# BioinformaticsArchive/POPBAM

Measured on AMD Instinct MI355X. Metric: Msites/sec (nucdiv+sfs+ld, 10kb win, 12 samples) at 1/2/4/8 GPUs, higher is better.
Workload: dtype f64; 1 GPU; configs[2]: synthetic 1 contig x 50 Msites x 12 samples per GPU, consensus call + nucdiv + sfs + ld(ZnS), 10 kb windows; sites_per_gpu=50000000, samples=12, mean_depth=10, window=10000, windows_per_gpu=4999, keys_per_gpu=6000082444, parallelism=dp1 (independent window-range shards, no collective), pieces=1

## Files before the change

popbam_amd/csrc/api.cpp:

```cpp
#include <dlfcn.h>
#include <hip/hip_runtime.h>

#include <algorithm>
#include <cmath>
#include <cstdlib>
#include <cstring>
#include <string>
#include <type_traits>
#include <vector>

#include "pbg_ctx.h"


namespace {

thread_local std::string g_create_error;

int fail(pbg_ctx *c, int code, const std::string &msg) {
    if (c) c->err = msg;
    else g_create_error = msg;
    return code;
}

}

int pbg::ctx_fail(pbg_ctx *c, int code, const std::string &msg) { return fail(c, code, msg); }

namespace {

#define HIPCHK(ctx, expr)                                                                          \
    do {                                                                                           \
        hipError_t _e = (expr);                                                                    \
        if (_e != hipSuccess)                                                                      \
            return fail((ctx), PBG_E_HIP, std::string(#expr) + ": " + hipGetErrorString(_e));      \
    } while (0)

uint32_t rms_of(uint32_t rmsq, int k) {
    const float f = (float)rmsq / (float)k;
    return (uint32_t)((double)std::sqrt(f) + 0.499);
}
uint32_t rms_threshold(int k, int min_rmsQ, int min_depth, int max_depth) {
    if (k < 1 || k < min_depth || k > max_depth) return 0xFFFFFFFFu;
    uint32_t lo = 0, hi = (uint32_t)k * 65025u;
    if ((int)rms_of(hi, k) < min_rmsQ) return 0xFFFFFFFFu;
    while (lo < hi) {
        const uint32_t mid = lo + (hi - lo) / 2;
        if ((int)rms_of(mid, k) >= min_rmsQ) hi = mid;
        else lo = mid + 1;
    }
    return lo;
}

int row_bytes_for(int n) { return n <= 14 ? 2 : n <= 30 ? 4 : n <= 62 ? 8 : 16; }

template <class T>
hipError_t upload(T **dst, const std::vector<T> &v) {
    hipError_t e = hipMalloc((void **)dst, std::max<size_t>(1, v.size()) * sizeof(T));
    if (e != hipSuccess) return e;
    if (v.empty()) return hipSuccess;
    return hipMemcpy(*dst, v.data(), v.size() * sizeof(T), hipMemcpyHostToDevice);
}


}

namespace {
std::vector<int32_t> jsfs_offsets(const pbg::DevParams &dp) {
    std::vector<int32_t> off;
    int32_t at = 0;
    for (int i = 0; i < dp.npops; ++i)
        for (int j = i + 1; j < dp.npops; ++j) {
            off.push_back(at);
            at += (dp.pop_n[i] + 1) * (dp.pop_n[j] + 1);
        }
    off.push_back(at);
    return off;
}

int check_pop_sizes(pbg_ctx *c, const char *what) {
    for (int i = 0; i < c->dp.npops; ++i)
        if (__builtin_popcountll(c->dp.pop_mask[i]) + __builtin_popcountll(c->dp.pop_mask_hi[i]) != c->dp.pop_n[i])
            return fail(c, PBG_E_ARG, std::string(what) + ": pop_n must be the number of samples in pop_mask");
    return PBG_OK;
// ... 187 lines not shown
                    for (uint32_t w = 0; w < 16; ++w)
                        fbeta[pbg::fbeta_index(q, nn, cc, w)] = q ? fk[w] * beta[q << 16 | nn << 8 | cc] : 0.0;
        if ((e = upload(&c->d_fbeta, fbeta)) != hipSuccess) return bad(e, "upload fbeta");
        std::vector<double> lb(pbg::kLbSize, 0.0);
        for (int m = 1; m <= 16; ++m) lb[m] = lb[m - 1] + fk[m - 1];
        for (int d = 3; d <= 16; ++d) {
            double run = 1e300;
            for (int q = 63; q >= 4; --q) {
                for (int cc = 0; cc <= d - 2; ++cc) run = std::min(run, beta[q << 16 | d << 8 | cc]);
                lb[17 + (q - 4) * 17 + d] = run;
            }
        }
        if ((e = upload(&c->d_lb, lb)) != hipSuccess) return bad(e, "upload lb");
        std::vector<double> oe(pbg::kOeSize, 0.0);
        for (int q = 4; q < 64; ++q)
            for (int d = 0; d <= 16; ++d) oe[(q - 4) * 17 + d] = beta[q << 16 | d << 8];
        for (int nn = 0; nn <= 16; ++nn)
            for (int kk = 0; kk <= 16; ++kk) oe[60 * 17 + nn * 17 + kk] = lhet[nn << 8 | kk];
        if ((e = upload(&c->d_oe, oe)) != hipSuccess) return bad(e, "upload one-error tables");
        {
            pbg::ScanTab st{};
            for (int q = 4; q < 64; ++q)
                for (int dd = 3; dd <= 16; ++dd) {
                    const volatile double pe = fk[0] * beta[q << 16 | dd << 8];
                    st.fpe[(q - 4) * 14 + dd - 3] = (float)pe;
                }
            for (int lev = 0; lev < 15; ++lev)
                for (int dd = 3; dd <= 16; ++dd) {
                    const double b = lb[17 + (4 * lev) * 17 + dd];
                    float f = (float)b;
                    if ((double)f > b) f = std::nextafter(f, 0.0f);
                    st.lq[lev * 14 + dd - 3] = f;
                }
            for (int dd = 3; dd <= 16; ++dd) {
                const int idx[4][2] = {{dd, dd - 1}, {dd, 1}, {dd - 1, 0}, {dd - 1, dd - 1}};
                for (int i = 0; i < 4; ++i) {
                    const volatile double h = -4.343 * lhet[idx[i][0] << 8 | idx[i][1]];
                    st.lh[(dd - 3) * 4 + i] = h;
                }
            }
            for (int m = 0; m <= 16; ++m) st.pre[m] = lb[m];
            if ((e = hipMalloc(&c->d_scantab, sizeof(st))) != hipSuccess) return bad(e, "hipMalloc scan tables");
            if ((e = hipMemcpy(c->d_scantab, &st, sizeof(st), hipMemcpyHostToDevice)) != hipSuccess)
                return bad(e, "upload scan tables");
        }
        std::vector<double> bu(60 * 17, 0.0);
        for (int dd = 1; dd <= 16; ++dd) {
            double run = 1e300;
            for (int q = 63; q >= 4; --q) {
                for (int cc = 0; cc <= dd - 1; ++cc) run = std::min(run, beta[q << 16 | dd << 8 | cc]);
                bu[(q - 4) * 17 + dd] = run;
            }
        }
        bool fk_dec = true;
        for (int w = 1; w < 16; ++w) fk_dec = fk_dec && fk[w] <= fk[w - 1];
        for (int i = 0; i < 17 * 3; ++i) d.uni[i] = 255u;
        for (int dd = 1; dd <= 16; ++dd) {
            float h[2];
            for (int t = 0; t < 2; ++t) {
                const float v = (float)(-4.343 * lhet[dd << 8 | (t ? dd : 0)]);
                h[t] = v < 0.0f ? 0.0f : v;
            }
            const float hm[3] = {h[0], h[1], std::min(h[0], h[1])};
            for (int cls = 0; cls < 3; ++cls) {
                uint32_t qthr = 255u;
                for (int q = 63; q >= 4; --q) {
                    const double lbv = lb[dd] * bu[(q - 4) * 17 + dd];
                    if (fk_dec && hm[cls] > 0.0f && lbv * (1.0 - 1e-9) > (double)hm[cls] * (1.0 + 1e-6) + 1e-3) qthr = (uint32_t)q;
                    else break;
                }
                const uint32_t snpq = (uint32_t)(uint64_t)((double)hm[cls] + 0.499) & 0xFFFFu;
                d.uni[dd * 3 + cls] = qthr | snpq << 8;
            }
        }
    }
    std::vector<double> a1, a2, e1, e2;
    pbg::build_sfs_constants(p->n_samples, a1, a2, e1, e2);
    const size_t L = a2.size();
    std::vector<double> sfs(4 * L, 0.0);
    std::copy(a1.begin(), a1.end(), sfs.begin());
    std::copy(a2.begin(), a2.end(), sfs.begin() + L);
    std::copy(e1.begin(), e1.end(), sfs.begin() + 2 * L);
    std::copy(e2.begin(), e2.end(), sfs.begin() + 3 * L);
    if ((e = upload(&c->d_sfs, sfs)) != hipSuccess) return bad(e, "upload sfs constants");
    std::vector<double> r2all;
    for (int i = 0; i < p->n_pops; ++i) {
        std::vector<double> t;
        pbg::build_r2_table(std::max(1, p->pop_n[i]), t);
        c->dt.r2_off[i] = (int32_t)r2all.size();
        r2all.insert(r2all.end(), t.begin(), t.end());
    }
    if ((e = upload(&c->d_r2, r2all)) != hipSuccess) return bad(e, "upload r2 tables");
    if ((e = hipMalloc(&c->d_err, sizeof(int))) != hipSuccess) return bad(e, "hipMalloc err");
    if ((e = hipMemset(c->d_err, 0, sizeof(int))) != hipSuccess) return bad(e, "hipMemset err");
    c->dt.fk = c->d_fk;
    c->dt.beta = c->d_beta;
    c->dt.lhet = c->d_lhet;
    c->dt.fbeta = c->d_fbeta;
    c->dt.lb = c->d_lb;
    c->dt.oe = c->d_oe;
    c->dt.scantab = reinterpret_cast<const uint4 *>(c->d_scantab);
    c->dt.a1 = c->d_sfs;
    c->dt.a2 = c->d_sfs + L;
    c->dt.e1 = c->d_sfs + 2 * L;
    c->dt.e2 = c->d_sfs + 3 * L;
    c->dt.r2 = c->d_r2;
// ... 658 lines not shown
```

popbam_amd/csrc/call_kernel.hip:

```cpp
#include <algorithm>

#include "pbg_common.h"

namespace pbg {
extern const int kBuildKind_call = PBG_BUILD_KIND;
}

namespace pbg {

namespace {

__device__ __forceinline__ unsigned char iupac_rev(unsigned char c) {
    switch (c) {
        case 'A': case 'a': return 0;
        case 'C': case 'c': return 1;
        case 'G': case 'g': return 2;
        case 'T': case 't': return 3;
        default: return 14;
    }
}
__device__ __forceinline__ char iupac_hom(unsigned g) {
    return g == 0 ? 'A' : g == 5 ? 'C' : g == 10 ? 'G' : 'T';
}
__device__ __forceinline__ uint32_t iupac_rev_bf(uint32_t c) {
    const uint32_t i = ((c & 0xDFu) - 'A') & 0xFFu;
    constexpr uint64_t kVal = (1ull << 4) | (2ull << 12) | (3ull << 38);
    constexpr uint32_t kOk = (1u << 0) | (1u << 2) | (1u << 6) | (1u << 19);
    const bool ok = i < 32u && ((kOk >> (i & 31u)) & 1u);
    return ok ? (uint32_t)(kVal >> (2u * (i & 31u))) & 3u : 14u;
}

__device__ __forceinline__ void cswap(uint32_t &a, uint32_t &b) {
    uint32_t hi = a > b ? a : b, lo = a > b ? b : a;
    a = hi;
    b = lo;
}
template <int N>
__device__ __forceinline__ void sortn_desc(uint32_t *k) {
#define CS(i, j) if constexpr ((j) < N) cswap(k[i], k[j])
    CS(0, 1); CS(2, 3); CS(0, 2); CS(1, 3); CS(1, 2); CS(4, 5); CS(6, 7); CS(4, 6);
    CS(5, 7); CS(5, 6); CS(0, 4); CS(2, 6); CS(2, 4); CS(1, 5); CS(3, 7); CS(3, 5);
    CS(1, 2); CS(3, 4); CS(5, 6);
    if constexpr (N <= 8) return;
    CS(8, 9); CS(10, 11); CS(8, 10); CS(9, 11); CS(9, 10);
    CS(12, 13); CS(14, 15); CS(12, 14); CS(13, 15); CS(13, 14); CS(8, 12); CS(10, 14); CS(10, 12);
    CS(9, 13); CS(11, 15); CS(11, 13); CS(9, 10); CS(11, 12); CS(13, 14); CS(0, 8); CS(4, 12);
    CS(4, 8); CS(2, 10); CS(6, 14); CS(6, 10); CS(2, 4); CS(6, 8); CS(10, 12); CS(1, 9);
    CS(5, 13); CS(5, 9); CS(3, 11); CS(7, 15); CS(7, 11); CS(3, 5); CS(7, 9); CS(11, 13);
    CS(1, 2); CS(3, 4); CS(5, 6); CS(7, 8); CS(9, 10); CS(11, 12); CS(13, 14);
#undef CS
}

__device__ __forceinline__ void sort32_desc(uint32_t *k) {
#define CS(i, j) cswap(k[i], k[j])
    CS(0, 1); CS(2, 3); CS(0, 2); CS(1, 3); CS(1, 2); CS(4, 5); CS(6, 7); CS(4, 6);
    CS(5, 7); CS(5, 6); CS(0, 4); CS(2, 6); CS(2, 4); CS(1, 5); CS(3, 7); CS(3, 5);
// ... 291 lines not shown
    a.bsum[0] = slot[0];
    a.bsum[1] = slot[SS];
    a.bsum[2] = slot[2 * SS];
    a.bsum[3] = slot[3 * SS];
    a.cpack = cvalid;
    a.wpack = 0;
    const uint64_t g = likelihood_gl2cns<LHS>(a, k, lhet);
    if constexpr (kRms) return g | rms_word((int)rmsq, k);
    else return g;
}

template <int LHS>
__device__ __forceinline__ uint64_t call_sample_reg(const uint32_t *rec, int d, int ng, uint32_t rmsq,
                                                    const double *__restrict__ fbeta, const double *lhet,
                                                    double *slot) {
    uint32_t key[16];
#pragma unroll
    for (int g = 0; g < 4; ++g) {
        if (g < 2 || g < ng) {
#pragma unroll
            for (int jj = 0; jj < 4; ++jj) {
                const int j = 4 * g + jj;
                const uint32_t v = rec[j < d ? j : 0];
                key[j] = j < d ? v : 0u;
            }
        } else {
#pragma unroll
            for (int jj = 0; jj < 4; ++jj) key[4 * g + jj] = 0u;
        }
    }
    return call_sample_words<LHS>(key, ng, d, rmsq, FbetaG{fbeta}, lhet, slot);
}

__device__ __forceinline__ uint32_t site_filters_rms(uint64_t &cb, unsigned char refc, const DevParams &P, bool rms_ok) {
    const uint32_t r = iupac_rev(refc);
    uint32_t lo = (uint32_t)cb;
    const uint32_t hi = (uint32_t)(cb >> 32);
    const uint32_t sq = hi & 0xffffu;
    const bool hq = (int)sq >= P.min_snpQ;
    if (!(P.flag & PBG_F_HETEROZYGOTE)) {
        const uint32_t g = (lo >> 8) & 0xffu;
        const uint32_t a1 = (g >> 2) & 3u, a2 = g & 3u;
        const uint32_t d = a2 - a1;
        const bool het = a1 != a2;
        const bool c1 = het && (hq ? a1 == r : a1 != r);
        const bool c2 = het && (hq ? a2 == r : a2 != r);
        lo += c1 ? d * 1024u : 0u;
        lo -= c2 ? d * 256u : 0u;
    }
    uint32_t info = 0;
    {
        const uint32_t g = (lo >> 8) & 0xffu;
        const uint32_t a1 = (g >> 2) & 3u, a2 = g & 3u;
        if (a1 == a2 && iupac_hom(g) != (char)refc) {
            if (hq) {
                lo |= 2u;
                info = 2u | (a1 << 2);
            } else {
                const uint32_t d = g - r;
                lo -= d * 256u;
                lo -= d * 1024u;
            }
        }
    }
    const uint32_t nr = lo >> 16;
    if (rms_ok && (int)nr >= P.min_depth && (int)nr <= P.max_depth) {
        lo |= 1u;
        info |= 1u;
    }
    cb = ((uint64_t)hi << 32) | lo;
    return info;
}
__device__ __forceinline__ uint32_t site_filters_rms_bf(uint64_t &cb, unsigned char refc, const DevParams &P, bool rms_ok) {
    const uint32_t r = iupac_rev_bf(refc);
    uint32_t lo = (uint32_t)cb;
    const uint32_t hi = (uint32_t)(cb >> 32);
    const uint32_t sq = hi & 0xffffu;
    const bool hq = (int)sq >= P.min_snpQ;
    if (!(P.flag & PBG_F_HETEROZYGOTE)) {
        const uint32_t g = (lo >> 8) & 0xffu;
        const uint32_t a1 = (g >> 2) & 3u, a2 = g & 3u;
        const uint32_t d = a2 - a1;
        const bool het = a1 != a2;
        const bool c1 = het && ((a1 == r) == hq);
        const bool c2 = het && ((a2 == r) == hq);
        lo += c1 ? d * 1024u : 0u;
        lo -= c2 ? d * 256u : 0u;
    }
    uint32_t info;
    {
        const uint32_t g = (lo >> 8) & 0xffu;
        const uint32_t a1 = (g >> 2) & 3u, a2 = g & 3u;
        const bool mis = a1 == a2 && !(r == a1 && (refc & 0x20u) == 0u);
        const uint32_t d = g - r;
        info = mis && hq ? 2u | (a1 << 2) : 0u;
        lo = !mis ? lo : hq ? lo | 2u : lo - d * 256u - d * 1024u;
    }
    const uint32_t nr = lo >> 16;
    const uint32_t pass = rms_ok && (int)nr >= P.min_depth && (int)nr <= P.max_depth ? 1u : 0u;
    lo |= pass;
    info |= pass;
    cb = ((uint64_t)hi << 32) | lo;
    return info;
}
__device__ __forceinline__ uint32_t site_filters(uint64_t &cb, unsigned char refc, const DevParams &P) {
// ... 410 lines not shown
                                         __builtin_elementwise_min(pk(v.z & M), pk(v.w & M)));
    };
    const pbg_u16x2 m = __builtin_elementwise_min(cmin(c0), __builtin_elementwise_min(cmin(u1 ? c1 : c0), cmin(u2 ? c2 : c0)));
    return (uint32_t)min(m.x, m.y) >> 5;
}
__device__ __forceinline__ uint32_t chunk_key(const uint4 &c0, const uint4 &c1, const uint4 &c2, uint32_t j) {
    const uint4 c = (j & 16u) ? c2 : (j & 8u) ? c1 : c0;
    const uint32_t lo = (j & 2u) ? c.y : c.x, hi = (j & 2u) ? c.w : c.z;
    const uint32_t w = (j & 4u) ? hi : lo;
    return (w >> ((j & 1u) * 16u)) & 0xFFFFu;
}
__device__ __forceinline__ bool one_error_ref(uint32_t bases, uint32_t strands, uint32_t qmin, uint32_t d, uint32_t r,
                                              const uint4 &c0, const uint4 &c1, const uint4 &c2, uint32_t sh,
                                              const double *beta0, const double *fk, const double *lb,
                                              const double *lhet, uint64_t &cb) {
    if (d < 3u || d > 16u) return false;
    const uint32_t vm2 = d >= 16u ? 0xFFFFFFFFu : (1u << (2u * d)) - 1u;
    const uint32_t pat = (r & 1u ? 0x55555555u : 0u) | (r & 2u ? 0xAAAAAAAAu : 0u);
    const uint32_t x = (bases ^ pat) & vm2;
    const uint32_t nz = (x | (x >> 1)) & 0x55555555u;
    if (__popc(nz) != 1) return false;
    const uint32_t ei = (uint32_t)__builtin_ctz(nz) >> 1;
    const uint32_t e = (bases >> (2u * ei)) & 3u;
    const uint32_t vm = d >= 16u ? 0xFFFFu : (1u << d) - 1u;
    const uint32_t n1 = (uint32_t)__popc(strands & vm & ~(1u << ei));
    const uint32_t n0 = d - 1u - n1;
    const uint32_t qe = min(max(chunk_key(c0, c1, c2, sh + ei) >> 5, 4u), 63u);
    const uint32_t ce = e < r ? d - 1u : 1u;
    const double t_be = beta0[(qe - 4u) * 17u + d], t_f0 = fk[0];
    const double t_he = lhet[d * 17u + ce], t_hz0 = lhet[(d - 1u) * 17u], t_hz1 = lhet[(d - 1u) * 17u + d - 1u];
    const double t_l0 = lb[n0], t_l1 = lb[n1], t_lq = lb[17 + (qmin - 4u) * 17u + d];
    const double pe = t_f0 * t_be;
    const float fpe = (float)pe;
    float v[4];
    uint32_t code[4];
    v[0] = fpe < 0.0f ? 0.0f : fpe;
    code[0] = r * 5u;
#pragma unroll
    for (uint32_t k = 1; k < 4; ++k) {
        const uint32_t y = (r + k) & 3u, lo = min(r, y), hi = max(r, y);
        const bool re = y == e;
        const double lh = -4.343 * (re ? t_he : (hi == r ? t_hz1 : t_hz0));
        const float val = re ? (float)lh : (float)(lh + (double)fpe);
        v[k] = val < 0.0f ? 0.0f : val;
        code[k] = (lo << 2) | hi;
    }
    const float mn = min(min(v[0], v[1]), min(v[2], v[3]));
    uint32_t min_ij = 16, ties = 0;
    float rest = 3.40282347e+38f;
#pragma unroll
    for (int k = 0; k < 4; ++k) {
        const bool eq = v[k] == mn;
        min_ij = eq ? min(min_ij, code[k]) : min_ij;
        ties += eq ? 1u : 0u;
        rest = eq ? rest : min(rest, v[k]);
    }
    const float mn_next = ties > 1u ? mn : rest;
    const double lbv = (t_l0 + t_l1) * t_lq;
    if (!(lbv * (1.0 - 1e-9) > (double)mn_next * (1.0 + 1e-6) + 1e-3)) return false;
    cb = ((uint64_t)((double)(mn_next - mn) + 0.499) << 32) + ((uint64_t)d << 16) + ((uint64_t)min_ij << 8);
    return true;
}
__device__ __forceinline__ bool one_error_ref_straight(uint32_t bases, uint32_t strands, uint32_t qmin, uint32_t d, uint32_t r,
                                                       const uint4 &c0, const uint4 &c1, const uint4 &c2, uint32_t sh,
                                                       const double *beta0, const double *fk, const double *lb,
                                                       const double *lhet, uint64_t &cb) {
    const uint32_t dd = min(max(d, 3u), 16u);
    const uint32_t vm2 = dd >= 16u ? 0xFFFFFFFFu : (1u << (2u * dd)) - 1u;
    const uint32_t pat = (r & 1u ? 0x55555555u : 0u) | (r & 2u ? 0xAAAAAAAAu : 0u);
    const uint32_t x = (bases ^ pat) & vm2;
    const uint32_t nz = (x | (x >> 1)) & 0x55555555u;
    const bool form = d == dd && __popc(nz) == 1;
    const uint32_t ei = min((uint32_t)__builtin_ctz(nz | 0x80000000u) >> 1, 15u);
    const uint32_t e = (bases >> (2u * ei)) & 3u;
    const uint32_t vm = dd >= 16u ? 0xFFFFu : (1u << dd) - 1u;
    const uint32_t n1 = min((uint32_t)__popc(strands & vm & ~(1u << ei)), dd - 1u);
    const uint32_t n0 = dd - 1u - n1;
    const uint32_t qe = min(max(chunk_key(c0, c1, c2, sh + ei) >> 5, 4u), 63u);
    const uint32_t ce = e < r ? dd - 1u : 1u;
#if defined(PBG_SCAN_EXP) && (PBG_SCAN_EXP & 32)
    const double t_be = beta0[dd & 1u], t_f0 = fk[0];
    const double t_he = lhet[ce & 1u], t_hz0 = lhet[2], t_hz1 = lhet[3];
    const double t_l0 = lb[n0 & 1u], t_l1 = lb[n1 & 1u], t_lq = lb[17 + (qmin & 1u)];
#else
    const double t_be = beta0[(qe - 4u) * 17u + dd], t_f0 = fk[0];
    const double t_he = lhet[dd * 17u + ce], t_hz0 = lhet[(dd - 1u) * 17u], t_hz1 = lhet[(dd - 1u) * 17u + dd - 1u];
    const double t_l0 = lb[n0], t_l1 = lb[n1], t_lq = lb[17 + (qmin - 4u) * 17u + dd];
#endif
    const double pe = t_f0 * t_be;
    const float fpe = (float)pe;
    float v[4];
    uint32_t code[4];
    v[0] = fpe < 0.0f ? 0.0f : fpe;
    code[0] = r * 5u;
#pragma unroll
    for (uint32_t k = 1; k < 4; ++k) {
        const uint32_t y = (r + k) & 3u, lo = min(r, y), hi = max(r, y);
        const bool re = y == e;
        const double lh = -4.343 * (re ? t_he : (hi == r ? t_hz1 : t_hz0));
        const float val = re ? (float)lh : (float)(lh + (double)fpe);
        v[k] = val < 0.0f ? 0.0f : val;
        code[k] = (lo << 2) | hi;
    }
    const float mn = min(min(v[0], v[1]), min(v[2], v[3]));
    uint32_t min_ij = 16, ties = 0;
    float rest = 3.40282347e+38f;
#pragma unroll
    for (int k = 0; k < 4; ++k) {
        const bool eq = v[k] == mn;
        min_ij = eq ? min(min_ij, code[k]) : min_ij;
        ties += eq ? 1u : 0u;
        rest = eq ? rest : min(rest, v[k]);
    }
    const float mn_next = ties > 1u ? mn : rest;
    const double lbv = (t_l0 + t_l1) * t_lq;
    cb = ((uint64_t)((double)(mn_next - mn) + 0.499) << 32) + ((uint64_t)dd << 16) + ((uint64_t)min_ij << 8);
    return form && lbv * (1.0 - 1e-9) > (double)mn_next * (1.0 + 1e-6) + 1e-3;
}

__device__ __forceinline__ bool one_error_ref_tab(uint32_t bases, uint32_t strands, uint32_t qmin, uint32_t d, uint32_t r,
                                                  const uint4 &c0, const uint4 &c1, const uint4 &c2, uint32_t sh,
                                                  const ScanTab &tab, uint64_t &cb) {
    const uint32_t dd = min(max(d, 3u), 16u);
    const uint32_t vm2 = dd >= 16u ? 0xFFFFFFFFu : (1u << (2u * dd)) - 1u;
    const uint32_t pat = (r & 1u ? 0x55555555u : 0u) | (r & 2u ? 0xAAAAAAAAu : 0u);
    const uint32_t x = (bases ^ pat) & vm2;
    const uint32_t nz = (x | (x >> 1)) & 0x55555555u;
    const bool form = d == dd && __popc(nz) == 1;
    const uint32_t ei = min((uint32_t)__builtin_ctz(nz | 0x80000000u) >> 1, 15u);
    const uint32_t e = (bases >> (2u * ei)) & 3u;
    const uint32_t vm = dd >= 16u ? 0xFFFFu : (1u << dd) - 1u;
    const uint32_t n1 = min((uint32_t)__popc(strands & vm & ~(1u << ei)), dd - 1u);
    const uint32_t n0 = dd - 1u - n1;
    const uint32_t qe = min(max(chunk_key(c0, c1, c2, sh + ei) >> 5, 4u), 63u);
    const float fpe = tab.fpe[(qe - 4u) * 14u + dd - 3u];
    const double *lh4 = tab.lh + (dd - 3u) * 4u;
    const double h_e = e < r ? lh4[0] : lh4[1];
    const double h_z0 = lh4[2], h_z1 = lh4[3];
    const double t_l0 = tab.pre[n0], t_l1 = tab.pre[n1];
    const double t_lq = (double)tab.lq[((qmin - 4u) >> 2) * 14u + dd - 3u];
    float v[4];
    uint32_t code[4];
    v[0] = fpe < 0.0f ? 0.0f : fpe;
    code[0] = r * 5u;
#pragma unroll
    for (uint32_t k = 1; k < 4; ++k) {
        const uint32_t y = (r + k) & 3u, lo = min(r, y), hi = max(r, y);
        const bool re = y == e;
        const double lh = re ? h_e : (hi == r ? h_z1 : h_z0);
        const float val = re ? (float)lh : (float)(lh + (double)fpe);
        v[k] = val < 0.0f ? 0.0f : val;
        code[k] = (lo << 2) | hi;
    }
    const float mn = min(min(v[0], v[1]), min(v[2], v[3]));
    uint32_t min_ij = 16, ties = 0;
    float rest = 3.40282347e+38f;
#pragma unroll
    for (int k = 0; k < 4; ++k) {
        const bool eq = v[k] == mn;
        min_ij = eq ? min(min_ij, code[k]) : min_ij;
        ties += eq ? 1u : 0u;
        rest = eq ? rest : min(rest, v[k]);
    }
    const float mn_next = ties > 1u ? mn : rest;
    const double lbv = (t_l0 + t_l1) * t_lq;
    cb = ((uint64_t)((double)(mn_next - mn) + 0.499) << 32) + ((uint64_t)dd << 16) + ((uint64_t)min_ij << 8);
    return form && lbv * (1.0 - 1e-9) > (double)mn_next * (1.0 + 1e-6) + 1e-3;
}

__device__ __forceinline__ bool uniform_ref(uint32_t qmin, uint32_t d, uint32_t m, const uint32_t *uni, uint64_t &cb) {
    if (d < 1u || d > 16u) return false;
    const uint32_t cls = m == 0u ? 0u : m == 3u ? 1u : 2u;
    const uint32_t e = uni[d * 3u + cls];
    if (qmin < (e & 255u)) return false;
    cb = ((uint64_t)(e >> 8) << 32) + ((uint64_t)d << 16) + ((uint64_t)(m * 5u) << 8);
    return true;
}
__device__ __forceinline__ bool uniform_ref_straight(uint32_t qmin, uint32_t d, uint32_t m, const uint32_t *uni, uint64_t &cb) {
    const uint32_t dd = min(max(d, 1u), 16u);
    const uint32_t cls = m == 0u ? 0u : m == 3u ? 1u : 2u;
    const uint32_t e = uni[dd * 3u + cls];
    cb = ((uint64_t)(e >> 8) << 32) + ((uint64_t)dd << 16) + ((uint64_t)(m * 5u) << 8);
    return d == dd && qmin >= (e & 255u);
}

__device__ __forceinline__ bool settle_packed(const uint4 &c0, const uint4 &c1, const uint4 &c2, uint32_t sh, uint32_t d,
                                              const uint32_t *uni, const DevTables &T,
                                              uint64_t &cb) {
    const bool n1 = sh + d > 8u, n2 = sh + d > 16u;
    const uint64_t b48 = (uint64_t)base_pack(c0) | ((uint64_t)base_pack(c1) << 16) | ((uint64_t)base_pack(c2) << 32);
    const uint32_t st = (strand_pack(c0) | (strand_pack(c1) << 8) | (strand_pack(c2) << 16)) >> sh;
    const uint32_t qm = chunk_qmin(c0, c1, c2, n1, n2);
    const uint32_t bs = (uint32_t)(b48 >> (2u * sh));
    const uint32_t vm2 = d >= 16u ? 0xFFFFFFFFu : (1u << (2u * d)) - 1u;
    const uint32_t m0 = bs & 3u;
    const uint32_t x0 = (bs ^ (m0 * 0x55555555u)) & vm2;
    const uint32_t c0n = (uint32_t)__popc((x0 | (x0 >> 1)) & 0x55555555u);
    const uint32_t mm = c0n + 1u == d && d >= 3u ? (bs >> 2) & 3u : m0;
    const uint32_t qb = max(qm, 4u);
    if (c0n == 0u) return uniform_ref(qb, d, m0, uni, cb);
    if (d >= 3u) return one_error_ref(bs, st, qb, d, mm, c0, c1, c2, sh, T.oe, T.fk, T.lb, T.oe + 60 * 17, cb);
    return false;
}

template <int BW, class Word>
__device__ __forceinline__ bool fold_position(int n, Word word, int rb, void *rows, size_t site) {
    int cnt[4] = {0, 0, 0, 0};
    int pass = 0;
    uint64_t types = 0, types_hi = 0;
    uint32_t queued = 0, first = 0;
    for (int j0 = 0; j0 < n; j0 += 4 * BW) {
        uint32_t wv[BW];
#pragma unroll
        for (int q = 0; q < BW; ++q) wv[q] = j0 + 4 * q < n ? word(j0 + 4 * q) : 0u;
        if (j0 == 0) first = wv[0];
// ... 168 lines not shown
            bool done = false;
            uint64_t cb = 0;
            uint32_t sh = 0;
            if constexpr (!kStraight) c0 = c1 = c2 = make_uint4(0, 0, 0, 0);
            if (haskeys) {
                const uint32_t a = koff >> 3;
                sh = koff & 7u;
                const bool tr = act && !deep && d >= 1u;
                const bool n1 = sh + d > 8u, n2 = sh + d > 16u;
                PBG_BOUNDS_CHUNK(B, ((gbase - galign) >> 3) + min(a, clast));
                PBG_BOUNDS_CHUNK(B, ((gbase - galign) >> 3) + min(n1 ? a + 1u : a, clast));
                PBG_BOUNDS_CHUNK(B, ((gbase - galign) >> 3) + min(n2 ? a + 2u : a, clast));
#if defined(PBG_SCAN_EXP) && (PBG_SCAN_EXP & 1)
                c0 = rd4[min(a, clast) & 7u];
                c1 = rd4[min(n1 ? a + 1u : a, clast) & 7u];
                c2 = rd4[min(n2 ? a + 2u : a, clast) & 7u];
#else
                if (f0 != 0u || (uint32_t)lane >= npre) {
                    c0 = rd4[min(a, clast)];
                    c1 = rd4[min(n1 ? a + 1u : a, clast)];
                    c2 = rd4[min(n2 ? a + 2u : a, clast)];
                }
#endif
                const uint64_t b48 = (uint64_t)base_pack(c0) | ((uint64_t)base_pack(c1) << 16) | ((uint64_t)base_pack(c2) << 32);
                const uint32_t st = (strand_pack(c0) | (strand_pack(c1) << 8) | (strand_pack(c2) << 16)) >> sh;
                const uint32_t qm = chunk_qmin(c0, c1, c2, n1, n2);
                const uint32_t bs = (uint32_t)(b48 >> (2u * sh));
                const uint32_t vm2 = d >= 16u ? 0xFFFFFFFFu : (1u << (2u * d)) - 1u;
                const uint32_t m0 = bs & 3u;
                const uint32_t x0 = (bs ^ (m0 * 0x55555555u)) & vm2;
                const uint32_t c0n = (uint32_t)__popc((x0 | (x0 >> 1)) & 0x55555555u);
                const uint32_t mm = c0n + 1u == d && d >= 3u ? (bs >> 2) & 3u : m0;
                const uint32_t qb = max(qm, 4u);
                if constexpr (kStraight) {
                    uint64_t cbu, cbo;
                    const bool du = uniform_ref_straight(qb, d, m0, uni, cbu);
#if defined(PBG_SCAN_EXP) && (PBG_SCAN_EXP & 16)
                    const bool dn = true;
                    cbo = bs;
#else
                    bool dn;
                    if constexpr (kTab) dn = one_error_ref_tab(bs, st, qb, d, mm, c0, c1, c2, sh, tab, cbo);
                    else dn = one_error_ref_straight(bs, st, qb, d, mm, c0, c1, c2, sh, T.oe, T.fk, T.lb, T.oe + 60 * 17, cbo);
#endif
                    done = tr && (c0n == 0u ? du : dn);
                    cb = c0n == 0u ? cbu : cbo;
                } else {
                    if (tr && c0n == 0u) done = uniform_ref(qb, d, m0, uni, cb);
                    else if (tr && d >= 3u) done = one_error_ref(bs, st, qb, d, mm, c0, c1, c2, sh, T.oe, T.fk, T.lb, T.oe + 60 * 17, cb);
                }
            }
            if constexpr (kStraight) {
                if (done) put1(t, site_filters_rms_bf(cb, (unsigned char)refw, P, rq >= rthr[d]) | 0x10u);
            } else {
                if (done) put1(t, site_filters_rms(cb, (unsigned char)refw, P, rq >= rthr[d]) | 0x10u);
            }
            const bool hard = act && !deep && !done;
            const uint64_t mh = __ballot(hard);
            if (mh) {
                const uint32_t ch = (uint32_t)__popcll(mh);
                const uint32_t ca = (uint32_t)max(0, min((int)ch, (int)qcap - (int)nq));
                const uint32_t rk = lane_rank(mh);
                if (hard) {
#if defined(PBG_SCAN_EXP) && (PBG_SCAN_EXP & 8)
                    if (false) {
#else
                    if (rk < ca) {
#endif
                        uint32_t wk[8];
                        task_words(c0, c1, c2, sh, d, wk);
                        uint4 *rec = qraw + 3u * (nq + rk);
                        const uint64_t ri = (uint64_t)blk * qcap * 3u + 3u * (nq + rk) + 2u;
                        (void)ri;
                        if (PBG_STORE_OK(err, ri, min((uint64_t)(blk + 1u) * qcap * 3u, D.raw_chk), D.raw_n, kErrQueue)) {
                            rec[0] = make_uint4(site0 + sl, smp | (d << 8), rq, refw & 0xFFu);
                            rec[1] = make_uint4(wk[0], wk[1], wk[2], wk[3]);
                            rec[2] = make_uint4(wk[4], wk[5], wk[6], wk[7]);
                        }
                    } else {
                        put1(t, 0x40u);
                    }
                }
                overflowed |= ca < ch;
                acc_s += ca;
                nq += ch;
// ... 1388 lines not shown
```

popbam_amd/csrc/pbg_common.h:

```cpp
#pragma once
#include <hip/hip_runtime.h>
#include <stdint.h>

#include "../../include/popbam_gpu.h"
#define PBG_HD __host__ __device__
#include "pbg_key.h"

#if !defined(PBG_EXPERIMENT)
#if defined(PBG_SLOW_NONET) || defined(PBG_ZNS_EXP) || defined(PBG_ZNS_SORT) || defined(PBG_ZNS_PRIO) || \
    defined(PBG_SCAN_WIDE_PASS) || defined(PBG_CALL_WAVES_PER_SIMD) || defined(PBG_SLOW_WG_PER_CU) ||      \
    defined(PBG_WIN_AHEAD) || defined(PBG_FAST_MAX) || defined(PBG_SYNTH_EXP) || defined(PBG_SCAN_EXP) || \
    defined(PBG_SCAN_LDS_PAD) || defined(PBG_ZNS_GROUPS) || defined(PBG_XPNSL_PLAIN)
#error "an experiment switch is defined: build variants with tools/variant.sh (-DPBG_EXPERIMENT=1)"
#endif
#define PBG_BUILD_KIND (PBG_BOUNDS_KIND)
#else
#define PBG_BUILD_KIND 2
#endif
#ifdef PBG_BOUNDS
#define PBG_BOUNDS_KIND 1
#else
#define PBG_BOUNDS_KIND 0
#endif

// ... 8 lines not shown
struct DevParams {
    int32_t n, npops;
    uint64_t pop_mask[PBG_MAX_POPS];
    uint64_t pop_mask_hi[PBG_MAX_POPS];
    int32_t pop_n[PBG_MAX_POPS];
    int32_t min_depth, max_depth, min_rmsQ, min_snpQ, min_mapQ, min_baseQ;
    uint32_t flag;
    int32_t k16;
    int32_t sfs_stride;
    int32_t pop_nmax;
    int32_t pops_ordered;
    int8_t sample_pop[PBG_MAX_SAMPLES];
    uint8_t pop_member[PBG_MAX_SAMPLES];
    int16_t pop_start[PBG_MAX_POPS + 1];
    uint32_t rms_thr[PBG_FAST_MAX + 1];
    uint32_t rmsq_thr[17];
    uint32_t uni[17 * 3];
};

struct DevTables {
    const double *fk;
    const double *beta;
    const double *lhet;
    const double *fbeta;
    const double *lb;
    const double *oe;
    const uint4 *scantab;
    const double *a1, *a2, *e1, *e2;
    const double *r2;
    int32_t r2_off[PBG_MAX_POPS];
};

constexpr int kLbSize = 17 + 60 * 17;
struct ScanTab {
    float fpe[60 * 14];
    float lq[15 * 14];
    double lh[14 * 4];
    double pre[17];
};
static_assert(sizeof(ScanTab) % 16 == 0, "ScanTab is copied as uint4");
constexpr int kScanTabVec = (int)(sizeof(ScanTab) / 16);
constexpr int kOeSize = 60 * 17 + 17 * 17;
constexpr int kFbetaN = 17;
__host__ __device__ inline uint32_t fbeta_index(uint32_t q, uint32_t n, uint32_t c, uint32_t w) {
    return ((q * kFbetaN + n) << 8) | (c << 4) | w;
}
constexpr size_t kFbetaSize = 64u * kFbetaN * 256u;

__host__ __device__ inline uint64_t splitmix64(uint64_t x) {
    uint64_t z = x + 0x9E3779B97F4A7C15ULL;
    z = (z ^ (z >> 30)) * 0xBF58476D1CE4E5B9ULL;
    z = (z ^ (z >> 27)) * 0x94D049BB133111EBULL;
    return z ^ (z >> 31);
}

struct SynthSite {
    uint64_t h;
    int ref_idx, alt, snp;
    uint32_t f16;
};
__host__ __device__ inline SynthSite synth_site_h(uint64_t h) {
    SynthSite s;
    s.h = h;
    s.ref_idx = (int)(s.h & 3);
    s.snp = ((s.h >> 2) & 0x3FF) < 12;
    s.alt = (s.ref_idx + 1 + (int)((((s.h >> 12) & 0xFFFFu) * 3u) >> 16)) & 3;
    s.f16 = (uint32_t)((s.h >> 16) & 0xFFFF);
    return s;
}
__host__ __device__ inline uint64_t synth_site_hash(uint64_t seed, int contig, uint64_t pos) {
    return splitmix64(seed ^ splitmix64(pos ^ ((uint64_t)(uint32_t)contig << 40)));
}
__host__ __device__ inline SynthSite synth_site(uint64_t seed, int contig, uint64_t pos) {
    SynthSite s;
// ... 337 lines not shown
```

Before: 13490 Msites/s.

## Precompute one-error and uniform site outcomes on host to skip per-site filter logic

The host now precomputes the site-filter outcome per (depth, ref, error base) for the one-error case, as a q-threshold step table in ScanTab, and packs a high-quality bit plus a depth-borrow mask into the uniform table. The tabled scan path then emits site info directly without building the full call word or running site_filters_rms. It falls back to the full one_error_ref_tab computation under a wave ballot when a case is not tabulated. This trims per-site ALU and double-precision work in the hot scan, at the cost of more complex host validation logic and a divergent fallback path.

```diff
diff --git a/popbam_amd/csrc/api.cpp b/popbam_amd/csrc/api.cpp
--- a/popbam_amd/csrc/api.cpp
+++ b/popbam_amd/csrc/api.cpp
@@ -49,6 +49,38 @@
         else lo = mid + 1;
     }
     return lo;
+}
+
+void one_error_outcomes(const pbg::DevParams &P, const std::vector<double> &lhet, pbg::ScanTab &st) {
+    for (int dd = 3; dd <= 16; ++dd) {
+        const volatile double hz0 = -4.343 * lhet[(dd - 1) << 8 | 0], hz1 = -4.343 * lhet[(dd - 1) << 8 | (dd - 1)];
+        const volatile double hlo = -4.343 * lhet[dd << 8 | (dd - 1)], hhi = -4.343 * lhet[dd << 8 | 1];
+        for (int i = 0; i < 2; ++i) {
+            const float v = (float)(i ? hhi : hlo);
+            st.he[(dd - 3) * 2 + i] = v < 0.0f ? 0.0f : v;
+        }
+        for (uint32_t r = 0; r < 4; ++r)
+            for (uint32_t e = 0; e < 4; ++e) {
+                uint8_t &step = st.step[(dd - 3) * 16 + r * 4 + e];
+                step = (uint8_t)pbg::kStepNone;
+                if (e == r) continue;
+                const float he = st.he[(dd - 3) * 2 + (e < r ? 0 : 1)];
+                bool ok = true;
+                int first = 64;
+                for (int q = 4; q < 64 && ok; ++q) {
+                    const float fpe = st.fpe[(q - 4) * 14 + dd - 3];
+                    float mn_next;
+                    uint64_t cb = pbg::one_error_word(fpe, e < r ? hlo : hhi, hz0, hz1, r, e, (uint32_t)dd, mn_next);
+                    const float v0 = fpe < 0.0f ? 0.0f : fpe;
+                    ok = mn_next == (v0 > he ? v0 : he);
+                    const uint32_t info = pbg::site_filters_rms(cb, (unsigned char)"ACGT"[r], P, true) & ~1u;
+                    ok = ok && (uint32_t)(cb >> 16 & 0xFFFFu) == (uint32_t)dd;
+                    if (info == (2u | e << 2)) first = std::min(first, q);
+                    else ok = ok && info == 0u && first == 64;
+                }
+                if (ok) step = (uint8_t)first;
+            }
+    }
 }
 
 int row_bytes_for(int n) { return n <= 14 ? 2 : n <= 30 ? 4 : n <= 62 ? 8 : 16; }
@@ -302,14 +334,8 @@
                     if ((double)f > b) f = std::nextafter(f, 0.0f);
                     st.lq[lev * 14 + dd - 3] = f;
                 }
-            for (int dd = 3; dd <= 16; ++dd) {
-                const int idx[4][2] = {{dd, dd - 1}, {dd, 1}, {dd - 1, 0}, {dd - 1, dd - 1}};
-                for (int i = 0; i < 4; ++i) {
-                    const volatile double h = -4.343 * lhet[idx[i][0] << 8 | idx[i][1]];
-                    st.lh[(dd - 3) * 4 + i] = h;
-                }
-            }
             for (int m = 0; m <= 16; ++m) st.pre[m] = lb[m];
+            one_error_outcomes(d, lhet, st);
             if ((e = hipMalloc(&c->d_scantab, sizeof(st))) != hipSuccess) return bad(e, "hipMalloc scan tables");
             if ((e = hipMemcpy(c->d_scantab, &st, sizeof(st), hipMemcpyHostToDevice)) != hipSuccess)
                 return bad(e, "upload scan tables");
@@ -340,8 +366,32 @@
                     else break;
                 }
                 const uint32_t snpq = (uint32_t)(uint64_t)((double)hm[cls] + 0.499) & 0xFFFFu;
-                d.uni[dd * 3 + cls] = qthr | snpq << 8;
-            }
+                d.uni[dd * 3 + cls] = qthr | snpq << 8 | ((int)snpq >= p->min_snpQ ? 1u << 24 : 0u);
+            }
+        }
+        {
+            uint32_t mask = 0;
+            bool ok = true;
+            for (int pass = 0; pass < 2; ++pass)
+                for (uint32_t dd = 1; dd <= 16; ++dd)
+                    for (uint32_t m = 0; m < 4; ++m)
+                        for (const char *rc = "ACGTacgtN"; *rc; ++rc) {
+                            const uint32_t cls = m == 0u ? 0u : m == 3u ? 1u : 2u, ue = d.uni[dd * 3 + cls];
+                            const bool hq = (ue >> 24) & 1u, mref = *rc == "ACGT"[m];
+                            const uint32_t v = *rc != 'N', bit = 1u << (m * 2u + v);
+                            uint64_t cb = ((uint64_t)((ue >> 8) & 0xFFFFu) << 32) + ((uint64_t)dd << 16) + ((uint64_t)(m * 5u) << 8);
+                            const uint32_t info = pbg::site_filters_rms(cb, (unsigned char)*rc, d, true) & ~1u;
+                            const uint32_t nr = (uint32_t)(cb >> 16) & 0xFFFFu;
+                            if (pass == 0) {
+                                if (!mref && !hq && nr != dd) mask |= bit;
+                            } else {
+                                const uint32_t bor = !mref && !hq && (mask & bit) ? 1u : 0u;
+                                ok = ok && nr == dd - bor && info == (!mref && hq ? 2u | m << 2 : 0u);
+                            }
+                        }
+            d.uni[0] = 255u | mask << 8;
+            if (!ok)
+                for (int i = 0; i < 17 * 3; ++i) d.uni[i] |= 255u;
         }
     }
     std::vector<double> a1, a2, e1, e2;
diff --git a/popbam_amd/csrc/call_kernel.hip b/popbam_amd/csrc/call_kernel.hip
--- a/popbam_amd/csrc/call_kernel.hip
+++ b/popbam_amd/csrc/call_kernel.hip
@@ -10,18 +10,6 @@
 
 namespace {
 
-__device__ __forceinline__ unsigned char iupac_rev(unsigned char c) {
-    switch (c) {
-        case 'A': case 'a': return 0;
-        case 'C': case 'c': return 1;
-        case 'G': case 'g': return 2;
-        case 'T': case 't': return 3;
-        default: return 14;
-    }
-}
-__device__ __forceinline__ char iupac_hom(unsigned g) {
-    return g == 0 ? 'A' : g == 5 ? 'C' : g == 10 ? 'G' : 'T';
-}
 __device__ __forceinline__ uint32_t iupac_rev_bf(uint32_t c) {
     const uint32_t i = ((c & 0xDFu) - 'A') & 0xFFu;
     constexpr uint64_t kVal = (1ull << 4) | (2ull << 12) | (3ull << 38);
@@ -379,45 +367,6 @@
     return call_sample_words<LHS>(key, ng, d, rmsq, FbetaG{fbeta}, lhet, slot);
 }
 
-__device__ __forceinline__ uint32_t site_filters_rms(uint64_t &cb, unsigned char refc, const DevParams &P, bool rms_ok) {
-    const uint32_t r = iupac_rev(refc);
-    uint32_t lo = (uint32_t)cb;
-    const uint32_t hi = (uint32_t)(cb >> 32);
-    const uint32_t sq = hi & 0xffffu;
-    const bool hq = (int)sq >= P.min_snpQ;
-    if (!(P.flag & PBG_F_HETEROZYGOTE)) {
-        const uint32_t g = (lo >> 8) & 0xffu;
-        const uint32_t a1 = (g >> 2) & 3u, a2 = g & 3u;
-        const uint32_t d = a2 - a1;
-        const bool het = a1 != a2;
-        const bool c1 = het && (hq ? a1 == r : a1 != r);
-        const bool c2 = het && (hq ? a2 == r : a2 != r);
-        lo += c1 ? d * 1024u : 0u;
-        lo -= c2 ? d * 256u : 0u;
-    }
-    uint32_t info = 0;
-    {
-        const uint32_t g = (lo >> 8) & 0xffu;
-        const uint32_t a1 = (g >> 2) & 3u, a2 = g & 3u;
-        if (a1 == a2 && iupac_hom(g) != (char)refc) {
-            if (hq) {
-                lo |= 2u;
-                info = 2u | (a1 << 2);
-            } else {
-                const uint32_t d = g - r;
-                lo -= d * 256u;
-                lo -= d * 1024u;
-            }
-        }
-    }
-    const uint32_t nr = lo >> 16;
-    if (rms_ok && (int)nr >= P.min_depth && (int)nr <= P.max_depth) {
-        lo |= 1u;
-        info |= 1u;
-    }
-    cb = ((uint64_t)hi << 32) | lo;
-    return info;
-}
 __device__ __forceinline__ uint32_t site_filters_rms_bf(uint64_t &cb, unsigned char refc, const DevParams &P, bool rms_ok) {
     const uint32_t r = iupac_rev_bf(refc);
     uint32_t lo = (uint32_t)cb;
@@ -894,33 +843,11 @@
     const double t_l0 = lb[n0], t_l1 = lb[n1], t_lq = lb[17 + (qmin - 4u) * 17u + d];
     const double pe = t_f0 * t_be;
     const float fpe = (float)pe;
-    float v[4];
-    uint32_t code[4];
-    v[0] = fpe < 0.0f ? 0.0f : fpe;
-    code[0] = r * 5u;
-#pragma unroll
-    for (uint32_t k = 1; k < 4; ++k) {
-        const uint32_t y = (r + k) & 3u, lo = min(r, y), hi = max(r, y);
-        const bool re = y == e;
-        const double lh = -4.343 * (re ? t_he : (hi == r ? t_hz1 : t_hz0));
-        const float val = re ? (float)lh : (float)(lh + (double)fpe);
-        v[k] = val < 0.0f ? 0.0f : val;
-        code[k] = (lo << 2) | hi;
-    }
-    const float mn = min(min(v[0], v[1]), min(v[2], v[3]));
-    uint32_t min_ij = 16, ties = 0;
-    float rest = 3.40282347e+38f;
-#pragma unroll
-    for (int k = 0; k < 4; ++k) {
-        const bool eq = v[k] == mn;
-        min_ij = eq ? min(min_ij, code[k]) : min_ij;
-        ties += eq ? 1u : 0u;
-        rest = eq ? rest : min(rest, v[k]);
-    }
-    const float mn_next = ties > 1u ? mn : rest;
+    float mn_next;
+    const uint64_t w = one_error_word(fpe, -4.343 * t_he, -4.343 * t_hz0, -4.343 * t_hz1, r, e, d, mn_next);
     const double lbv = (t_l0 + t_l1) * t_lq;
     if (!(lbv * (1.0 - 1e-9) > (double)mn_next * (1.0 + 1e-6) + 1e-3)) return false;
-    cb = ((uint64_t)((double)(mn_next - mn) + 0.499) << 32) + ((uint64_t)d << 16) + ((uint64_t)min_ij << 8);
+    cb = w;
     return true;
 }
 __device__ __forceinline__ bool one_error_ref_straight(uint32_t bases, uint32_t strands, uint32_t qmin, uint32_t d, uint32_t r,
@@ -951,83 +878,67 @@
 #endif
     const double pe = t_f0 * t_be;
     const float fpe = (float)pe;
-    float v[4];
-    uint32_t code[4];
-    v[0] = fpe < 0.0f ? 0.0f : fpe;
-    code[0] = r * 5u;
-#pragma unroll
-    for (uint32_t k = 1; k < 4; ++k) {
-        const uint32_t y = (r + k) & 3u, lo = min(r, y), hi = max(r, y);
-        const bool re = y == e;
-        const double lh = -4.343 * (re ? t_he : (hi == r ? t_hz1 : t_hz0));
-        const float val = re ? (float)lh : (float)(lh + (double)fpe);
-        v[k] = val < 0.0f ? 0.0f : val;
-        code[k] = (lo << 2) | hi;
-    }
-    const float mn = min(min(v[0], v[1]), min(v[2], v[3]));
-    uint32_t min_ij = 16, ties = 0;
-    float rest = 3.40282347e+38f;
-#pragma unroll
-    for (int k = 0; k < 4; ++k) {
-        const bool eq = v[k] == mn;
-        min_ij = eq ? min(min_ij, code[k]) : min_ij;
-        ties += eq ? 1u : 0u;
-        rest = eq ? rest : min(rest, v[k]);
-    }
-    const float mn_next = ties > 1u ? mn : rest;
+    float mn_next;
+    const uint64_t w = one_error_word(fpe, -4.343 * t_he, -4.343 * t_hz0, -4.343 * t_hz1, r, e, dd, mn_next);
     const double lbv = (t_l0 + t_l1) * t_lq;
-    cb = ((uint64_t)((double)(mn_next - mn) + 0.499) << 32) + ((uint64_t)dd << 16) + ((uint64_t)min_ij << 8);
+    cb = w;
     return form && lbv * (1.0 - 1e-9) > (double)mn_next * (1.0 + 1e-6) + 1e-3;
 }
 
-__device__ __forceinline__ bool one_error_ref_tab(uint32_t bases, uint32_t strands, uint32_t qmin, uint32_t d, uint32_t r,
-                                                  const uint4 &c0, const uint4 &c1, const uint4 &c2, uint32_t sh,
-                                                  const ScanTab &tab, uint64_t &cb) {
+struct OneErrKeys {
+    bool form;
+    uint32_t dd, e;
+    float fpe;
+    double lbv;
+};
+__device__ __forceinline__ OneErrKeys one_error_keys(uint32_t bases, uint32_t strands, uint32_t qmin, uint32_t d, uint32_t r,
+                                                     const uint4 &c0, const uint4 &c1, const uint4 &c2, uint32_t sh,
+                                                     const ScanTab &tab, uint32_t &qe) {
+    OneErrKeys k;
     const uint32_t dd = min(max(d, 3u), 16u);
     const uint32_t vm2 = dd >= 16u ? 0xFFFFFFFFu : (1u << (2u * dd)) - 1u;
     const uint32_t pat = (r & 1u ? 0x55555555u : 0u) | (r & 2u ? 0xAAAAAAAAu : 0u);
     const uint32_t x = (bases ^ pat) & vm2;
     const uint32_t nz = (x | (x >> 1)) & 0x55555555u;
-    const bool form = d == dd && __popc(nz) == 1;
+    k.form = d == dd && __popc(nz) == 1;
     const uint32_t ei = min((uint32_t)__builtin_ctz(nz | 0x80000000u) >> 1, 15u);
-    const uint32_t e = (bases >> (2u * ei)) & 3u;
+    k.e = (bases >> (2u * ei)) & 3u;
+    k.dd = dd;
     const uint32_t vm = dd >= 16u ? 0xFFFFu : (1u << dd) - 1u;
     const uint32_t n1 = min((uint32_t)__popc(strands & vm & ~(1u << ei)), dd - 1u);
     const uint32_t n0 = dd - 1u - n1;
-    const uint32_t qe = min(max(chunk_key(c0, c1, c2, sh + ei) >> 5, 4u), 63u);
-    const float fpe = tab.fpe[(qe - 4u) * 14u + dd - 3u];
-    const double *lh4 = tab.lh + (dd - 3u) * 4u;
-    const double h_e = e < r ? lh4[0] : lh4[1];
-    const double h_z0 = lh4[2], h_z1 = lh4[3];
+    qe = min(max(chunk_key(c0, c1, c2, sh + ei) >> 5, 4u), 63u);
+    k.fpe = tab.fpe[(qe - 4u) * 14u + dd - 3u];
     const double t_l0 = tab.pre[n0], t_l1 = tab.pre[n1];
     const double t_lq = (double)tab.lq[((qmin - 4u) >> 2) * 14u + dd - 3u];
-    float v[4];
-    uint32_t code[4];
-    v[0] = fpe < 0.0f ? 0.0f : fpe;
-    code[0] = r * 5u;
-#pragma unroll
-    for (uint32_t k = 1; k < 4; ++k) {
-        const uint32_t y = (r + k) & 3u, lo = min(r, y), hi = max(r, y);
-        const bool re = y == e;
-        const double lh = re ? h_e : (hi == r ? h_z1 : h_z0);
-        const float val = re ? (float)lh : (float)(lh + (double)fpe);
-        v[k] = val < 0.0f ? 0.0f : val;
-        code[k] = (lo << 2) | hi;
-    }
-    const float mn = min(min(v[0], v[1]), min(v[2], v[3]));
-    uint32_t min_ij = 16, ties = 0;
-    float rest = 3.40282347e+38f;
-#pragma unroll
-    for (int k = 0; k < 4; ++k) {
-        const bool eq = v[k] == mn;
-        min_ij = eq ? min(min_ij, code[k]) : min_ij;
-        ties += eq ? 1u : 0u;
-        rest = eq ? rest : min(rest, v[k]);
-    }
-    const float mn_next = ties > 1u ? mn : rest;
-    const double lbv = (t_l0 + t_l1) * t_lq;
-    cb = ((uint64_t)((double)(mn_next - mn) + 0.499) << 32) + ((uint64_t)dd << 16) + ((uint64_t)min_ij << 8);
-    return form && lbv * (1.0 - 1e-9) > (double)mn_next * (1.0 + 1e-6) + 1e-3;
+    k.lbv = (t_l0 + t_l1) * t_lq;
+    return k;
+}
+__device__ __forceinline__ bool one_error_ref_tab(uint32_t bases, uint32_t strands, uint32_t qmin, uint32_t d, uint32_t r,
+                                                  const uint4 &c0, const uint4 &c1, const uint4 &c2, uint32_t sh,
+                                                  const ScanTab &tab, const double *lhet, uint64_t &cb) {
+    uint32_t qe;
+    const OneErrKeys k = one_error_keys(bases, strands, qmin, d, r, c0, c1, c2, sh, tab, qe);
+    const uint32_t dd = k.dd;
+    const double t_he = lhet[dd * 17u + (k.e < r ? dd - 1u : 1u)];
+    const double t_hz0 = lhet[(dd - 1u) * 17u], t_hz1 = lhet[(dd - 1u) * 17u + dd - 1u];
+    float mn_next;
+    cb = one_error_word(k.fpe, -4.343 * t_he, -4.343 * t_hz0, -4.343 * t_hz1, r, k.e, dd, mn_next);
+    return k.form && k.lbv * (1.0 - 1e-9) > (double)mn_next * (1.0 + 1e-6) + 1e-3;
+}
+__device__ __forceinline__ bool one_error_outcome(uint32_t bases, uint32_t strands, uint32_t qmin, uint32_t d, uint32_t r,
+                                                  const uint4 &c0, const uint4 &c1, const uint4 &c2, uint32_t sh,
+                                                  const ScanTab &tab, bool isref, bool &other, uint32_t &out) {
+    uint32_t qe;
+    const OneErrKeys k = one_error_keys(bases, strands, qmin, d, r, c0, c1, c2, sh, tab, qe);
+    const float he = tab.he[(k.dd - 3u) * 2u + (k.e < r ? 0u : 1u)];
+    const uint32_t stp = tab.step[(k.dd - 3u) * 16u + r * 4u + k.e];
+    const float v0 = k.fpe < 0.0f ? 0.0f : k.fpe;
+    const float mn_next = fmaxf(v0, he);
+    const bool tabbed = isref && stp != kStepNone;
+    other = k.form && !tabbed;
+    out = qe >= stp ? 2u | (k.e << 2) : 0u;
+    return k.form && tabbed && k.lbv * (1.0 - 1e-9) > (double)mn_next * (1.0 + 1e-6) + 1e-3;
 }
 
 __device__ __forceinline__ bool uniform_ref(uint32_t qmin, uint32_t d, uint32_t m, const uint32_t *uni, uint64_t &cb) {
@@ -1035,14 +946,28 @@
     const uint32_t cls = m == 0u ? 0u : m == 3u ? 1u : 2u;
     const uint32_t e = uni[d * 3u + cls];
     if (qmin < (e & 255u)) return false;
-    cb = ((uint64_t)(e >> 8) << 32) + ((uint64_t)d << 16) + ((uint64_t)(m * 5u) << 8);
+    cb = ((uint64_t)((e >> 8) & 0xFFFFu) << 32) + ((uint64_t)d << 16) + ((uint64_t)(m * 5u) << 8);
     return true;
 }
 __device__ __forceinline__ bool uniform_ref_straight(uint32_t qmin, uint32_t d, uint32_t m, const uint32_t *uni, uint64_t &cb) {
     const uint32_t dd = min(max(d, 1u), 16u);
     const uint32_t cls = m == 0u ? 0u : m == 3u ? 1u : 2u;
     const uint32_t e = uni[dd * 3u + cls];
-    cb = ((uint64_t)(e >> 8) << 32) + ((uint64_t)dd << 16) + ((uint64_t)(m * 5u) << 8);
+    cb = ((uint64_t)((e >> 8) & 0xFFFFu) << 32) + ((uint64_t)dd << 16) + ((uint64_t)(m * 5u) << 8);
+    return d == dd && qmin >= (e & 255u);
+}
+
+__device__ __forceinline__ bool uniform_outcome(uint32_t qmin, uint32_t d, uint32_t m, const uint32_t *uni, uint32_t refw,
+                                                bool rms_ok, const DevParams &P, uint32_t &out) {
+    const uint32_t dd = min(max(d, 1u), 16u);
+    const uint32_t cls = m == 0u ? 0u : m == 3u ? 1u : 2u;
+    const uint32_t e = uni[dd * 3u + cls];
+    const bool mref = (refw >> 8) == m + 1u, hq = (e >> 24) & 1u;
+    const uint32_t v = iupac_rev_bf(refw & 0xFFu) != 14u ? 1u : 0u;
+    const uint32_t bor = !mref && !hq ? (uni[0] >> (8u + m * 2u + v)) & 1u : 0u;
+    const int nr = (int)(d - bor);
+    const uint32_t pass = rms_ok && nr >= P.min_depth && nr <= P.max_depth ? 1u : 0u;
+    out = pass | (!mref && hq ? 2u | (m << 2) : 0u);
     return d == dd && qmin >= (e & 255u);
 }
 
@@ -1277,16 +1202,32 @@
                 const uint32_t c0n = (uint32_t)__popc((x0 | (x0 >> 1)) & 0x55555555u);
                 const uint32_t mm = c0n + 1u == d && d >= 3u ? (bs >> 2) & 3u : m0;
                 const uint32_t qb = max(qm, 4u);
-                if constexpr (kStraight) {
+                if constexpr (kTab) {
+                    bool other;
+                    uint32_t ob;
+                    const bool isref = (refw >> 8) == mm + 1u;
+                    const bool dn = one_error_outcome(bs, st, qb, d, mm, c0, c1, c2, sh, tab, isref, other, ob);
+                    uint32_t ub;
+                    const bool du = uniform_outcome(qb, d, m0, uni, refw, rq >= rthr[d], P, ub);
+                    if (tr && (c0n == 0u ? du : dn)) {
+                        put1(t, (c0n == 0u ? ub : (rq >= thr[d] ? 1u : 0u) | ob) | 0x10u);
+                        done = true;
+                    }
+                    const bool rest = tr && other;
+                    if (__ballot(rest)) {
+                        if (one_error_ref_tab(bs, st, qb, d, mm, c0, c1, c2, sh, tab, T.oe + 60 * 17, cb) && rest) {
+                            put1(t, site_filters_rms_bf(cb, (unsigned char)refw, P, rq >= rthr[d]) | 0x10u);
+                            done = true;
+                        }
+                    }
+                } else if constexpr (kStraight) {
                     uint64_t cbu, cbo;
                     const bool du = uniform_ref_straight(qb, d, m0, uni, cbu);
 #if defined(PBG_SCAN_EXP) && (PBG_SCAN_EXP & 16)
                     const bool dn = true;
                     cbo = bs;
 #else
-                    bool dn;
-                    if constexpr (kTab) dn = one_error_ref_tab(bs, st, qb, d, mm, c0, c1, c2, sh, tab, cbo);
-                    else dn = one_error_ref_straight(bs, st, qb, d, mm, c0, c1, c2, sh, T.oe, T.fk, T.lb, T.oe + 60 * 17, cbo);
+                    const bool dn = one_error_ref_straight(bs, st, qb, d, mm, c0, c1, c2, sh, T.oe, T.fk, T.lb, T.oe + 60 * 17, cbo);
 #endif
                     done = tr && (c0n == 0u ? du : dn);
                     cb = c0n == 0u ? cbu : cbo;
@@ -1295,7 +1236,8 @@
                     else if (tr && d >= 3u) done = one_error_ref(bs, st, qb, d, mm, c0, c1, c2, sh, T.oe, T.fk, T.lb, T.oe + 60 * 17, cb);
                 }
             }
-            if constexpr (kStraight) {
+            if constexpr (kTab) {
+            } else if constexpr (kStraight) {
                 if (done) put1(t, site_filters_rms_bf(cb, (unsigned char)refw, P, rq >= rthr[d]) | 0x10u);
             } else {
                 if (done) put1(t, site_filters_rms(cb, (unsigned char)refw, P, rq >= rthr[d]) | 0x10u);
diff --git a/popbam_amd/csrc/pbg_common.h b/popbam_amd/csrc/pbg_common.h
--- a/popbam_amd/csrc/pbg_common.h
+++ b/popbam_amd/csrc/pbg_common.h
@@ -64,14 +64,100 @@
 };
 
 constexpr int kLbSize = 17 + 60 * 17;
+constexpr uint32_t kStepNone = 0xFFu;
 struct ScanTab {
     float fpe[60 * 14];
     float lq[15 * 14];
-    double lh[14 * 4];
+    float he[14 * 2];
+    uint8_t step[14 * 16];
+    uint8_t unused[112];
     double pre[17];
 };
+static_assert(sizeof(ScanTab) == 4784, "ScanTab must not grow (LDS of the n <= 12 scan)");
 static_assert(sizeof(ScanTab) % 16 == 0, "ScanTab is copied as uint4");
 constexpr int kScanTabVec = (int)(sizeof(ScanTab) / 16);
+
+PBG_HD __forceinline__ uint64_t one_error_word(float fpe, double h_e, double h_z0, double h_z1, uint32_t r, uint32_t e,
+                                               uint32_t d, float &mn_next) {
+    float v[4];
+    uint32_t code[4];
+    v[0] = fpe < 0.0f ? 0.0f : fpe;
+    code[0] = r * 5u;
+#pragma unroll
+    for (uint32_t k = 1; k < 4; ++k) {
+        const uint32_t y = (r + k) & 3u, lo = r < y ? r : y, hi = r < y ? y : r;
+        const bool re = y == e;
+        const double lh = re ? h_e : (hi == r ? h_z1 : h_z0);
+        const float val = re ? (float)lh : (float)(lh + (double)fpe);
+        v[k] = val < 0.0f ? 0.0f : val;
+        code[k] = (lo << 2) | hi;
+    }
+    const float mn = fminf(fminf(v[0], v[1]), fminf(v[2], v[3]));
+    uint32_t min_ij = 16, ties = 0;
+    float rest = 3.40282347e+38f;
+#pragma unroll
+    for (int k = 0; k < 4; ++k) {
+        const bool eq = v[k] == mn;
+        min_ij = eq ? (min_ij < code[k] ? min_ij : code[k]) : min_ij;
+        ties += eq ? 1u : 0u;
+        rest = eq ? rest : fminf(rest, v[k]);
+    }
+    mn_next = ties > 1u ? mn : rest;
+    return ((uint64_t)((double)(mn_next - mn) + 0.499) << 32) + ((uint64_t)d << 16) + ((uint64_t)min_ij << 8);
+}
+
+PBG_HD __forceinline__ unsigned char iupac_rev(unsigned char c) {
+    switch (c) {
+        case 'A': case 'a': return 0;
+        case 'C': case 'c': return 1;
+        case 'G': case 'g': return 2;
+        case 'T': case 't': return 3;
+        default: return 14;
+    }
+}
+PBG_HD __forceinline__ char iupac_hom(unsigned g) {
+    return g == 0 ? 'A' : g == 5 ? 'C' : g == 10 ? 'G' : 'T';
+}
+
+PBG_HD __forceinline__ uint32_t site_filters_rms(uint64_t &cb, unsigned char refc, const DevParams &P, bool rms_ok) {
+    const uint32_t r = iupac_rev(refc);
+    uint32_t lo = (uint32_t)cb;
+    const uint32_t hi = (uint32_t)(cb >> 32);
+    const uint32_t sq = hi & 0xffffu;
+    const bool hq = (int)sq >= P.min_snpQ;
+    if (!(P.flag & PBG_F_HETEROZYGOTE)) {
+        const uint32_t g = (lo >> 8) & 0xffu;
+        const uint32_t a1 = (g >> 2) & 3u, a2 = g & 3u;
+        const uint32_t d = a2 - a1;
+        const bool het = a1 != a2;
+        const bool c1 = het && (hq ? a1 == r : a1 != r);
+        const bool c2 = het && (hq ? a2 == r : a2 != r);
+        lo += c1 ? d * 1024u : 0u;
+        lo -= c2 ? d * 256u : 0u;
+    }
+    uint32_t info = 0;
+    {
+        const uint32_t g = (lo >> 8) & 0xffu;
+        const uint32_t a1 = (g >> 2) & 3u, a2 = g & 3u;
+        if (a1 == a2 && iupac_hom(g) != (char)refc) {
+            if (hq) {
+                lo |= 2u;
+                info = 2u | (a1 << 2);
+            } else {
+                const uint32_t d = g - r;
+                lo -= d * 256u;
+                lo -= d * 1024u;
+            }
+        }
+    }
+    const uint32_t nr = lo >> 16;
+    if (rms_ok && (int)nr >= P.min_depth && (int)nr <= P.max_depth) {
+        lo |= 1u;
+        info |= 1u;
+    }
+    cb = ((uint64_t)hi << 32) | lo;
+    return info;
+}
 constexpr int kOeSize = 60 * 17 + 17 * 17;
 constexpr int kFbetaN = 17;
 __host__ __device__ inline uint32_t fbeta_index(uint32_t q, uint32_t n, uint32_t c, uint32_t w) {
```

New measurement: 13470 Msites/s. No clear change (-0.1%).
